# pocokhc/simple_distributed_rl

Measured on AMD Instinct MI355X. Metric: env-steps/sec + learner updates/sec, Rainbow 84x84x4, higher is better.
Workload: dtype f32

## Files before the change

### simple_distributed_rl_amd/csrc/srlx_qnet_bwd.hip

```cpp
#include <new>

#include "srlx_adam_math.h"
#include "srlx_qnet_int.h"
#include "srlx_td_math.h"

namespace {

using i64 = int64_t;
using u8 = unsigned char;
using f32x16 = __attribute__((ext_vector_type(16))) float;

constexpr int kFcSplits = 16;
constexpr int kWgSplits = 64;
constexpr int kC1Pad = 88, kC1Frame = kC1Pad * kC1Pad, kC1Chunks = 4;

__device__ __forceinline__ int clampi(int v, int lo, int hi) { return v < lo ? lo : (v > hi ? hi : v); }
__device__ __forceinline__ float byte_to_unit(unsigned b) {
    const float x = (float)b, rcp = 1.0f / 255.0f;
    const float q = x * rcp;
    return fmaf(fmaf(-q, 255.0f, x), rcp, q);
}

template <int AMAX>
__global__ void __launch_bounds__(256) k_head_bwd(int B, i64 sstride, int hidden, int A, int dueling, const float *dq,
                                                   const float *__restrict__ h1, const float *__restrict__ v2w, const float *__restrict__ a2w,
                                                   float *__restrict__ dh1, float *__restrict__ dh1t , float *__restrict__ g_bf,
                                                   float *__restrict__ g_v2w, float *__restrict__ g_v2b, float *__restrict__ g_a2w, float *__restrict__ g_a2b,
                                                   srlx::TdArgs td, int with_td) {
    extern __shared__ __attribute__((aligned(16))) float sm[];
    float *dv = sm, *da = sm + B, *part = sm + B + B * A;
    if (with_td) {
        float *sdq = part + (3 + AMAX) * 256;
        int off = B + 2 * B * A + (3 + AMAX) * 256;
        off += off & 1;
        double *red = reinterpret_cast<double *>(sm + off);
        const int t = threadIdx.x;
        const double la = srlx::td_rows(td, t, 256, sdq, blockIdx.x == 0);
        if (blockIdx.x == 0) {
            red[t] = la;
            __syncthreads();
            for (int s = 128; s > 0; s >>= 1) {
                if (t < s) red[t] += red[t + s];
                __syncthreads();
            }
            if (t == 0) td.loss[0] = (float)(red[0] / (double)td.B);
        }
        __syncthreads();
        dq = sdq;
    }
    for (int b = threadIdx.x; b < B; b += blockDim.x) {
        float s = 0.f;
        for (int j = 0; j < A; j++) s += dq[b * A + j];
        dv[b] = s;
        for (int j = 0; j < A; j++) da[b * A + j] = dueling == 0 ? dq[b * A + j] - s / (float)A : dq[b * A + j];
    }
    __syncthreads();
    const int ul = threadIdx.x & 63, slice = threadIdx.x >> 6;
    const int u = blockIdx.x * 64 + ul;
    const int N1 = 2 * hidden;
    float gv = 0.f, gbv = 0.f, gba = 0.f, ga[AMAX];
#pragma unroll
    for (int j = 0; j < AMAX; j++) ga[j] = 0.f;
    if (u < hidden) {
        const float wv = v2w[u];
        float wa[AMAX];
#pragma unroll
        for (int j = 0; j < AMAX; j++) wa[j] = j < A ? a2w[j * hidden + u] : 0.f;
#pragma unroll 8
        for (int b = slice; b < B; b += 4) {
            const float hv = h1[(i64)b * sstride * N1 + u], ha = h1[(i64)b * sstride * N1 + hidden + u];
            gv += dv[b] * hv;
            float s = 0.f;
#pragma unroll
            for (int j = 0; j < AMAX; j++)
                if (j < A) {
                    ga[j] += da[b * A + j] * ha;
                    s += da[b * A + j] * wa[j];
                }
            const float dhv = hv > 0.f ? dv[b] * wv : 0.f, dha = ha > 0.f ? s : 0.f;
            dh1[(i64)b * N1 + u] = dhv;
            dh1[(i64)b * N1 + hidden + u] = dha;
            if (dh1t) dh1t[u * 32 + b] = dhv, dh1t[(hidden + u) * 32 + b] = dha;
            gbv += dhv;
            gba += dha;
        }
        if (dh1t)
            for (int b = slice; b < 32; b += 4)
                if (b >= B) dh1t[u * 32 + b] = 0.f, dh1t[(hidden + u) * 32 + b] = 0.f;
    }
    part[0 * 256 + threadIdx.x] = gv;
    part[1 * 256 + threadIdx.x] = gbv;
    part[2 * 256 + threadIdx.x] = gba;
#pragma unroll
    for (int j = 0; j < AMAX; j++)
        if (j < A) part[(3 + j) * 256 + threadIdx.x] = ga[j];
    __syncthreads();
    if (slice == 0 && u < hidden) {
        auto sum4 = [&](int row) { return ((part[row * 256 + ul] + part[row * 256 + 64 + ul]) + part[row * 256 + 128 + ul]) + part[row * 256 + 192 + ul]; };
        g_v2w[u] = sum4(0);
        g_bf[u] = sum4(1);
        g_bf[hidden + u] = sum4(2);
#pragma unroll
        for (int j = 0; j < AMAX; j++)
            if (j < A) g_a2w[j * hidden + u] = sum4(3 + j);
    }
    if (blockIdx.x == 0 && threadIdx.x <= A) {
        float s = 0.f;
        if (threadIdx.x == A) {
            for (int b = 0; b < B; b++) s += dv[b];
            g_v2b[0] = s;
        } else {
            for (int b = 0; b < B; b++) s += da[b * A + threadIdx.x];
            g_a2b[threadIdx.x] = s;
        }
    }
}

__global__ void __launch_bounds__(256) k_uvfa_wgrad(int B, i64 sstride, int N1, int X, srlx_uvfa_dev uv, const float *__restrict__ dh1, float *__restrict__ g_wx) {
    const int id = blockIdx.x * 256 + threadIdx.x;
    if (id >= X * N1) return;
    const int c = id / N1, u = id % N1;
    float s = 0.f;
    for (int b = 0; b < B; b++) {
        const i64 row = (i64)b * sstride;
        float x;
        if (c == uv.c_ext) x = uv.r_ext[row];
        else if (c == uv.c_int) x = uv.r_int[row];
        else if (uv.c_act >= 0 && c >= uv.c_act && c < uv.c_act + uv.n_act_in) x = uv.action[row] == c - uv.c_act ? 1.f : 0.f;
        else x = (uv.c_actor >= 0 && uv.actor[row] == c - uv.c_actor) ? 1.f : 0.f;
        s += dh1[(i64)b * N1 + u] * x;
    }
    g_wx[id] = s;
}

template <int AMAX>
__global__ void __launch_bounds__(256) k_head_plain_bwd(int B, i64 sstride, int N1, int A, const float *__restrict__ dq, const float *__restrict__ h1,
                                                         const float *__restrict__ w2, float *__restrict__ dh1, float *__restrict__ dh1t ,
                                                         float *__restrict__ g_bf, float *__restrict__ g_w2, float *__restrict__ g_b2, srlx::TdArgs td, int with_td) {
    extern __shared__ __attribute__((aligned(16))) float sm[];
    float *part = sm, *sdq = sm + (1 + AMAX) * 256;
    const int t = threadIdx.x;
    if (with_td) {
        int off = (1 + AMAX) * 256 + B * A;
        off += off & 1;
        double *red = reinterpret_cast<double *>(sm + off);
        const double la = srlx::td_rows(td, t, 256, sdq, blockIdx.x == 0);
        if (blockIdx.x == 0) {
            red[t] = la;
            __syncthreads();
            for (int s = 128; s > 0; s >>= 1) {
                if (t < s) red[t] += red[t + s];
                __syncthreads();
            }
            if (t == 0) td.loss[0] = (float)(red[0] / (double)td.B);
        }
// ... 9 lines not shown
    if (u < N1) {
        float wa[AMAX];
#pragma unroll
        for (int j = 0; j < AMAX; j++) wa[j] = j < A ? w2[(i64)j * N1 + u] : 0.f;
#pragma unroll 4
        for (int b = slice; b < B; b += 4) {
            const float hv = h1[(i64)b * sstride * N1 + u];
            float s = 0.f;
#pragma unroll
            for (int j = 0; j < AMAX; j++)
                if (j < A) {
                    const float d = sdq[b * A + j];
                    ga[j] += d * hv;
                    s += d * wa[j];
                }
            const float dh = hv > 0.f ? s : 0.f;
            dh1[(i64)b * N1 + u] = dh;
            if (dh1t) dh1t[u * 32 + b] = dh;
            gb += dh;
        }
        if (dh1t)
            for (int b = slice; b < 32; b += 4)
                if (b >= B) dh1t[u * 32 + b] = 0.f;
    }
    part[t] = gb;
#pragma unroll
    for (int j = 0; j < AMAX; j++)
        if (j < A) part[(1 + j) * 256 + t] = ga[j];
    __syncthreads();
    if (slice == 0 && u < N1) {
        auto sum4 = [&](int row) { return ((part[row * 256 + ul] + part[row * 256 + 64 + ul]) + part[row * 256 + 128 + ul]) + part[row * 256 + 192 + ul]; };
        g_bf[u] = sum4(0);
#pragma unroll
        for (int j = 0; j < AMAX; j++)
            if (j < A) g_w2[(i64)j * N1 + u] = sum4(1 + j);
    }
    if (blockIdx.x == 0 && t < A) {
        float s = 0.f;
        for (int b = 0; b < B; b++) s += sdq[b * A + t];
        g_b2[t] = s;
    }
}

__global__ void __launch_bounds__(256) k_hidden_bwd(int B, i64 sstride, int N1, int out_cols, const float *__restrict__ g, const float *__restrict__ h1,
                                                    float *__restrict__ dh1, float *__restrict__ dh1t, float *__restrict__ g_bf) {
    __shared__ float part[256];
    const int ul = threadIdx.x & 63, slice = threadIdx.x >> 6;
    const int u = blockIdx.x * 64 + ul;
    float gb = 0.f;
    if (u < N1) {
        for (int b = slice; b < B; b += 4) {
            const float hv = h1[(i64)b * sstride * N1 + u];
            const float d = (u < out_cols && hv > 0.f) ? g[(i64)b * out_cols + u] : 0.f;
            dh1[(i64)b * N1 + u] = d;
            if (dh1t) dh1t[u * 32 + b] = d;
            gb += d;
        }
        if (dh1t)
            for (int b = slice; b < 32; b += 4)
                if (b >= B) dh1t[u * 32 + b] = 0.f;
    }
    part[threadIdx.x] = gb;
    __syncthreads();
    if (slice == 0 && u < N1) g_bf[u] = ((part[ul] + part[64 + ul]) + part[128 + ul]) + part[192 + ul];
}

template <bool ADAM, bool PLANES = false>
__global__ void __launch_bounds__(256) k_fc1_wgrad(int B, i64 sstride, int N1, int K, const float *__restrict__ dh1, const float *__restrict__ act3,
                                                   float *__restrict__ g_wf, float *__restrict__ wf, float *__restrict__ m, float *__restrict__ v, double lr, double beta1,
                                                   double beta2, double eps, const i64 *__restrict__ d_step, _Float16 *__restrict__ planes = nullptr) {
    const int lane = threadIdx.x & 63, i = lane & 31, h = lane >> 5;
    const int k0 = (blockIdx.x * 4 + (threadIdx.x >> 6)) * 32, n0 = blockIdx.y * 32;
    if (k0 >= K) return;
    float pp[16], mm[16], vv[16];
    if (ADAM)
#pragma unroll
        for (int r = 0; r < 16; r++) {
            const i64 at = (i64)(n0 + (r & 3) + 8 * (r >> 2) + 4 * h) * K + k0 + i;
            pp[r] = wf[at], mm[r] = m[at], vv[r] = v[at];
        }
    f32x16 acc;
#pragma unroll
    for (int r = 0; r < 16; r++) acc[r] = 0.f;
    const float *pa = dh1 + (i64)h * N1 + n0 + i, *pb = act3 + (i64)h * sstride * K + k0 + i;
    const int steps = (B + 1) / 2;
    for (int s0 = 0; s0 < steps; s0 += 8) {
        float av[8], bv[8];
#pragma unroll
        for (int q = 0; q < 8; q++) {
            const bool live = 2 * (s0 + q) + h < B;
            av[q] = live ? pa[(i64)(s0 + q) * 2 * N1] : 0.f;
            bv[q] = live ? pb[(i64)(s0 + q) * 2 * sstride * K] : 0.f;
        }
#pragma unroll
        for (int q = 0; q < 8; q++) acc = __builtin_amdgcn_mfma_f32_32x32x2f32(av[q], bv[q], acc, 0, 0, 0);
    }
    if (ADAM) {
        const srlx::AdamCoef c = srlx::adam_coef(lr, beta1, beta2, eps, *d_step);
#pragma unroll
        for (int r = 0; r < 16; r++) {
            const i64 at = (i64)(n0 + (r & 3) + 8 * (r >> 2) + 4 * h) * K + k0 + i;
            srlx::adam_one(pp[r], acc[r], mm[r], vv[r], c);
            wf[at] = pp[r], m[at] = mm[r], v[at] = vv[r];
            if (PLANES) {
                _Float16 *row = planes + (((i64)(k0 >> 5) * N1 + n0 + (r & 3) + 8 * (r >> 2) + 4 * h) * 64) + i;
                const _Float16 hi = (_Float16)pp[r];
                row[0] = hi;
                row[32] = (_Float16)((pp[r] - (float)hi) * 2048.0f);
            }
        }
    } else {
#pragma unroll
        for (int r = 0; r < 16; r++) g_wf[(i64)(n0 + (r & 3) + 8 * (r >> 2) + 4 * h) * K + k0 + i] = acc[r];
    }
}

template <int BT>
__global__ void __launch_bounds__(256) k_fc1_dgrad(int B, int N1, int K, const float *__restrict__ dh1, const float *__restrict__ wf, float *__restrict__ part) {
    __shared__ float sd[BT * 64];
    const int per = N1 / kFcSplits;
    const int n0 = blockIdx.y * per;
    const int k = blockIdx.x * 256 + threadIdx.x;
    for (int idx = threadIdx.x; idx < BT * per; idx += 256) {
        const int b = idx / per, nn = idx % per;
        sd[b * 64 + nn] = b < B ? dh1[(i64)b * N1 + n0 + nn] : 0.f;
    }
    __syncthreads();
    if (k >= K) return;
    float acc[BT];
#pragma unroll
    for (int b = 0; b < BT; b++) acc[b] = 0.f;
#pragma unroll 8
    for (int nn = 0; nn < per; nn++) {
        const float w = wf[(i64)(n0 + nn) * K + k];
#pragma unroll
        for (int b = 0; b < BT; b++) acc[b] += sd[b * 64 + nn] * w;
    }
#pragma unroll
    for (int b = 0; b < BT; b++)
        if (b < B) part[((i64)blockIdx.y * B + b) * K + k] = acc[b];
}

__global__ void __launch_bounds__(256) k_fc1_dgrad_reduce(int B, i64 sstride, int K, const float *__restrict__ part, const float *__restrict__ act3,
                                                          float *__restrict__ dact3) {
    const unsigned i = blockIdx.x * 256u + threadIdx.x;
    if (i >= (unsigned)(B * K)) return;
    const int b = (int)(i / (unsigned)K), k = (int)(i % (unsigned)K);
    float s = 0.f;
#pragma unroll
    for (int sp = 0; sp < kFcSplits; sp++) s += part[((i64)sp * B + b) * K + k];
    dact3[i] = act3[(i64)b * sstride * K + k] > 0.f ? s : 0.f;
}

__global__ void __launch_bounds__(256) k_fc1_dgrad_mfma(int B, i64 sstride, int N1, int K, const float *__restrict__ dh1t, const float *__restrict__ wf,
                                                        const float *__restrict__ act3, float *__restrict__ dact3) {
    __shared__ float red[3][16][64];
    const int t = threadIdx.x, wave = t >> 6, lane = t & 63, i = lane & 31, h = lane >> 5;
    const int k0 = blockIdx.x * 32;
    const int per = N1 / 4;
    const float *pa = dh1t + ((i64)wave * per + h) * 32 + i;
    const float *pb = wf + ((i64)wave * per + h) * K + k0 + i;
    f32x16 acc;
#pragma unroll
    for (int r = 0; r < 16; r++) acc[r] = 0.f;
    float a0[8], b0[8], a1[8], b1[8];
    auto fetch = [&](float *a, float *b, int s0) {
#pragma unroll
        for (int q = 0; q < 8; q++) {
            a[q] = pa[(i64)(s0 + q) * 64];
            b[q] = pb[(i64)(s0 + q) * 2 * K];
        }
    };
    const int steps = per / 2;
    fetch(a0, b0, 0);
    for (int s0 = 0; s0 < steps; s0 += 16) {
        if (s0 + 8 < steps) fetch(a1, b1, s0 + 8);
        __builtin_amdgcn_sched_barrier(0);
#pragma unroll
        for (int q = 0; q < 8; q++) acc = __builtin_amdgcn_mfma_f32_32x32x2f32(a0[q], b0[q], acc, 0, 0, 0);
        __builtin_amdgcn_sched_barrier(0);
        if (s0 + 8 >= steps) break;
        if (s0 + 16 < steps) fetch(a0, b0, s0 + 16);
        __builtin_amdgcn_sched_barrier(0);
#pragma unroll
        for (int q = 0; q < 8; q++) acc = __builtin_amdgcn_mfma_f32_32x32x2f32(a1[q], b1[q], acc, 0, 0, 0);
        __builtin_amdgcn_sched_barrier(0);
    }
    if (wave > 0)
#pragma unroll
        for (int r = 0; r < 16; r++) red[wave - 1][r][lane] = acc[r];
    __syncthreads();
    if (wave == 0)
#pragma unroll
        for (int r = 0; r < 16; r++) {
            const int b = (r & 3) + 8 * (r >> 2) + 4 * h;
            if (b < B) {
                const float sum = ((acc[r] + red[0][r][lane]) + red[1][r][lane]) + red[2][r][lane];
                dact3[(i64)b * K + k0 + i] = act3[(i64)b * sstride * K + k0 + i] > 0.f ? sum : 0.f;
            }
        }
}

struct ConvGeo {
    int H, W, CI, OH, OW, CO, KH, KW, S, P;
};
template <int CI>
__global__ void __launch_bounds__(256) k_conv_wgrad_mfma(ConvGeo g, i64 sstride, const float *__restrict__ X, const float *__restrict__ dY, float *__restrict__ part,
                                                         float *__restrict__ bias_part ) {
    constexpr int NCI = CI / 32, CO = 64;
    const int lane = threadIdx.x & 63, i = lane & 31, h = lane >> 5;
    const int combo = blockIdx.x * 4 + (threadIdx.x >> 6), taps = g.KH * g.KW;
    if (combo >= taps * 2 * NCI) return;
    const int cit = combo % NCI, cot = (combo / NCI) & 1, tap = combo / (2 * NCI);
    const int ky = tap / g.KW, kx = tap % g.KW;
    const i64 b = blockIdx.y;
    const int per_img = g.OH * g.OW, steps = (per_img + 1) / 2;
    const float *pa = dY + b * per_img * CO + cot * 32 + i;
    const float *px = X + b * sstride * g.H * g.W * CI + cit * 32 + i;
    int m = h, oy = 0, ox = h;
    f32x16 acc;
#pragma unroll
    for (int r = 0; r < 16; r++) acc[r] = 0.f;
    float bsum = 0.f;
    float a0[8], x0[8], a1[8], x1[8];
    auto fetch = [&](float *a, float *x) __attribute__((always_inline)) {
#pragma unroll
        for (int q = 0; q < 8; q++) {
            const bool live = m < per_img;
            const int iy = clampi(oy * g.S + ky - g.P, 0, g.H - 1), ix = clampi(ox * g.S + kx - g.P, 0, g.W - 1);
            a[q] = live ? pa[(i64)m * CO] : 0.f;
            x[q] = live ? px[((i64)iy * g.W + ix) * CI] : 0.f;
            m += 2, ox += 2;
            if (ox >= g.OW) ox -= g.OW, oy++;
        }
    };
    auto mfma8 = [&](const float *a, const float *x) __attribute__((always_inline)) {
#pragma unroll
        for (int q = 0; q < 8; q++) {
            bsum += a[q];
            acc = __builtin_amdgcn_mfma_f32_32x32x2f32(a[q], x[q], acc, 0, 0, 0);
        }
    };
    fetch(a0, x0);
    for (int s0 = 0; s0 < steps; s0 += 16) {
        if (s0 + 8 < steps) fetch(a1, x1);
        __builtin_amdgcn_sched_barrier(0);
        mfma8(a0, x0);
        __builtin_amdgcn_sched_barrier(0);
        if (s0 + 8 >= steps) break;
        if (s0 + 16 < steps) fetch(a0, x0);
        __builtin_amdgcn_sched_barrier(0);
        mfma8(a1, x1);
        __builtin_amdgcn_sched_barrier(0);
    }
#pragma unroll
    for (int r = 0; r < 16; r++) {
        const int co = cot * 32 + (r & 3) + 8 * (r >> 2) + 4 * h;
        part[((b * CO + co) * taps + tap) * CI + cit * 32 + i] = acc[r];
    }
    if (tap == 0 && cit == 0) {
        const float tot = bsum + __shfl_xor(bsum, 32);
        if (h == 0) bias_part[b * CO + cot * 32 + i] = tot;
    }
}

struct AdamArgs {
    double lr, beta1, beta2, eps;
    const i64 *d_step;
};
template <bool ADAM>
__global__ void __launch_bounds__(256) k_reduce_parts(const float *__restrict__ part, int P, i64 n, float *__restrict__ out, const float *__restrict__ bpart, int nb,
                                                      float *__restrict__ bout, float *__restrict__ pw = nullptr, float *__restrict__ mw = nullptr,
                                                      float *__restrict__ vw = nullptr, float *__restrict__ pb = nullptr, float *__restrict__ mb = nullptr,
                                                      float *__restrict__ vb = nullptr, AdamArgs ad = AdamArgs{}, i64 *__restrict__ snap = nullptr) {
    __shared__ float4 sm[4][64];
    const int lane = threadIdx.x & 63, sl = threadIdx.x >> 6;
    i64 i = ((i64)blockIdx.x * 64 + lane) * 4;
    const bool live = i < n + nb;
    if (ADAM && snap && blockIdx.x == 0 && threadIdx.x == 0) *snap = *ad.d_step;
    if (i >= n) {
        i -= n;
        part = bpart;
        n = nb;
        out = bout;
        pw = pb, mw = mb, vw = vb;
    }
    float4 pp, mm, vv;
    i64 step = 0;
    if (ADAM && sl == 0 && live) {
        pp = *reinterpret_cast<const float4 *>(pw + i), mm = *reinterpret_cast<const float4 *>(mw + i), vv = *reinterpret_cast<const float4 *>(vw + i);
        step = *ad.d_step;
    }
    const int per = (P + 3) / 4, p_lo = sl * per, p_hi = p_lo + per < P ? p_lo + per : P;
    float4 s = make_float4(0.f, 0.f, 0.f, 0.f);
    if (live)
#pragma unroll 8
        for (int p = p_lo; p < p_hi; p++) {
            const float4 v = *reinterpret_cast<const float4 *>(part + (i64)p * n + i);
            s.x += v.x, s.y += v.y, s.z += v.z, s.w += v.w;
        }
    sm[sl][lane] = s;
    __syncthreads();
    if (sl == 0 && live) {
        const float4 a = sm[1][lane], b = sm[2][lane], c = sm[3][lane];
        const float4 g = make_float4(((s.x + a.x) + b.x) + c.x, ((s.y + a.y) + b.y) + c.y, ((s.z + a.z) + b.z) + c.z, ((s.w + a.w) + b.w) + c.w);
        *reinterpret_cast<float4 *>(out + i) = g;
        if (ADAM) {
            const srlx::AdamCoef cf = srlx::adam_coef(ad.lr, ad.beta1, ad.beta2, ad.eps, step);
            srlx::adam_one(pp.x, g.x, mm.x, vv.x, cf);
            srlx::adam_one(pp.y, g.y, mm.y, vv.y, cf);
            srlx::adam_one(pp.z, g.z, mm.z, vv.z, cf);
            srlx::adam_one(pp.w, g.w, mm.w, vv.w, cf);
            *reinterpret_cast<float4 *>(pw + i) = pp;
            *reinterpret_cast<float4 *>(mw + i) = mm;
            *reinterpret_cast<float4 *>(vw + i) = vv;
        }
    }
}

__global__ void __launch_bounds__(256) k_transpose_filter(const float *__restrict__ W, int CO, int KH, int KW, int S, int CI, float *__restrict__ wT) {
    const int i = blockIdx.x * 256 + threadIdx.x;
    const int taps = KH * KW;
    if (i >= CO * taps * CI) return;
    const int ci = i % CI, tap = (i / CI) % taps, co = i / (CI * taps);
    const int ky = tap / KW, kx = tap % KW, KWS = KW / S, Kc = (KH / S) * KWS * CO;
    const int cls = (ky % S) * S + (kx % S);
    wT[((i64)cls * CI + ci) * Kc + ((ky / S) * KWS + kx / S) * CO + co] = W[i];
}

__global__ void __launch_bounds__(256) k_fold_pad(int B, i64 sstride, int H, int W, int CI, int P, int HP, int WP, int S, int QH, int QW,
                                                  const float *__restrict__ dxq, const float *__restrict__ X, float *__restrict__ dX, int nsplit = 1, i64 split_stride = 0) {
    const unsigned i4 = blockIdx.x * 256u + threadIdx.x;
    const unsigned c4n = (unsigned)CI / 4u;
    if (i4 >= (unsigned)(B * H * W) * c4n) return;
    const unsigned uw = (unsigned)W, uh = (unsigned)H;
    const int ci = 4 * (int)(i4 % c4n), ix = (int)((i4 / c4n) % uw), iy = (int)((i4 / (c4n * uw)) % uh), b = (int)(i4 / (c4n * uw * uh));
    const int y0 = iy == 0 ? 0 : iy + P, y1 = iy == H - 1 ? HP - 1 : iy + P;
    const int x0 = ix == 0 ? 0 : ix + P, x1 = ix == W - 1 ? WP - 1 : ix + P;
    const i64 cls_stride = (i64)B * QH * QW * CI;
    float4 s = make_float4(0.f, 0.f, 0.f, 0.f);
    for (int py = y0; py <= y1; py++)
        for (int px = x0; px <= x1; px++) {
            const float *src = dxq + ((py % S) * S + px % S) * cls_stride + (((i64)b * QH + py / S) * QW + px / S) * CI + ci;
            float4 v = *reinterpret_cast<const float4 *>(src);
            for (int sp = 1; sp < nsplit; sp++) {
                const float4 w = *reinterpret_cast<const float4 *>(src + sp * split_stride);
                v.x += w.x, v.y += w.y, v.z += w.z, v.w += w.w;
            }
            s.x += v.x, s.y += v.y, s.z += v.z, s.w += v.w;
        }
    const float4 x = *reinterpret_cast<const float4 *>(X + (((i64)b * sstride * H + iy) * W + ix) * CI + ci);
    *reinterpret_cast<float4 *>(dX + (i64)i4 * 4) = make_float4(x.x > 0.f ? s.x : 0.f, x.y > 0.f ? s.y : 0.f, x.z > 0.f ? s.z : 0.f, x.w > 0.f ? s.w : 0.f);
}

// ... 253 lines not shown
}

static int conv_chain(srlx_qnet_t *h, int B, i64 ss, const uint8_t *d_frame_base, const int64_t *d_frame_off, float *const *g, hipStream_t st, bool with_fc1) {
    const int N1 = 2 * h->hidden, K = h->flat, C2 = 2 * h->F1;
    float *g_w1 = g[0], *g_b1 = g[1], *g_w2 = g[2], *g_b2 = g[3], *g_w3 = g[4], *g_b3 = g[5], *g_wf = with_fc1 ? g[6] : nullptr;
    float *bias_part = h->w_part + h->w_part_floats;
    const size_t c3 = (size_t)2 * h->F1 * 9 * 2 * h->F1, c2 = (size_t)2 * h->F1 * 16 * h->F1;
    hipStream_t sd = h->side;
    SRLX_HIP(hipEventRecord(h->ev_d3, st));
    {
        const int HP = h->OH2 + 2, WP = h->OW2 + 2;
        const int nsplit = (C2 == 64 && h->dgrad_split == 2) ? 2 : 1;
        SRLX_TRY(srlx_qnet_dgrad_gemm(h->dact3, B, HP, WP, h->OH3, h->OW3, C2, 3, 3, 1, h->w_t, C2, h->dxpad, st, nsplit));
        const i64 tot = (i64)B * h->OH2 * h->OW2 * C2;
        hipLaunchKernelGGL(k_fold_pad, dim3((unsigned)((tot / 4 + 255) / 256)), dim3(256), 0, st, B, ss, h->OH2, h->OW2, C2, 1, HP, WP, 1, HP, WP, h->dxpad, h->act2, h->dact2, nsplit,
                           (i64)B * HP * WP * C2);
    }
    SRLX_STAMP(18, st);
    SRLX_HIP(hipEventRecord(h->ev_d2, st));
    {
        const int HP = h->OH1 + 4, WP = h->OW1 + 4, QH = (HP + 1) / 2, QW = (WP + 1) / 2;
        SRLX_TRY(srlx_qnet_dgrad_gemm(h->dact2, B, QH, QW, h->OH2, h->OW2, C2, 4, 4, 2, h->w_t2, h->F1, h->dxpad, st));
        const i64 tot = (i64)B * h->OH1 * h->OW1 * h->F1;
        hipLaunchKernelGGL(k_fold_pad, dim3((unsigned)((tot / 4 + 255) / 256)), dim3(256), 0, st, B, ss, h->OH1, h->OW1, h->F1, 2, HP, WP, 2, QH, QW, h->dxpad, h->act1, h->dact1);
    }
    SRLX_STAMP(19, st);
    SRLX_HIP(hipEventRecord(h->ev_d1, st));
    const dim3 fg((unsigned)((K / 32 + 3) / 4), (unsigned)(N1 / 32));
    if (with_fc1 && !h->adam_m)
        hipLaunchKernelGGL(k_fc1_wgrad<false>, fg, dim3(256), 0, sd, B, ss, N1, K, h->dh1, h->act3, g_wf, nullptr, nullptr, nullptr, 0.0, 0.0, 0.0, 0.0, nullptr);
    SRLX_HIP(hipStreamWaitEvent(sd, h->ev_d3, 0));
    const int fc1_order = h->fc1_order;
    auto launch_fc1_adam = [&](hipStream_t s2) {
        if (h->adam_planes_out)
            hipLaunchKernelGGL((k_fc1_wgrad<true, true>), fg, dim3(256), 0, s2, B, ss, N1, K, h->dh1, h->act3, nullptr, const_cast<float *>(h->wf), h->adam_m, h->adam_v,
                               h->adam_lr, h->adam_b1, h->adam_b2, h->adam_eps, h->adam_step, (_Float16 *)h->adam_planes_out);
        else
            hipLaunchKernelGGL(k_fc1_wgrad<true>, fg, dim3(256), 0, s2, B, ss, N1, K, h->dh1, h->act3, nullptr, const_cast<float *>(h->wf), h->adam_m, h->adam_v, h->adam_lr,
                               h->adam_b1, h->adam_b2, h->adam_eps, h->adam_step);
    };
    const bool fc1_adam = with_fc1 && h->adam_m;
    if (fc1_adam && fc1_order == 1) launch_fc1_adam(sd);
    if (fc1_adam && fc1_order == 2) {
        if (!h->side2) SRLX_HIP(hipStreamCreateWithFlags(&h->side2, hipStreamNonBlocking));
        SRLX_HIP(hipStreamWaitEvent(h->side2, h->ev_d3, 0));
        launch_fc1_adam(h->side2);
        SRLX_HIP(hipEventRecord(h->ev_join2, h->side2));
    }
    ConvGeo g3{h->OH2, h->OW2, C2, h->OH3, h->OW3, C2, 3, 3, 1, 1};
    hipLaunchKernelGGL(k_conv_wgrad_mfma<64>, dim3((9 * 2 * 2 + 3) / 4, (unsigned)B), dim3(256), 0, sd, g3, ss, h->act2, h->dact3, h->w_part, bias_part);
    const bool rest = h->rest_on && with_fc1;
    const AdamArgs ad{h->adam_lr, h->adam_b1, h->adam_b2, h->adam_eps, h->adam_step};
    auto reduce = [&](hipStream_t s_, const float *part_, int P_, i64 n_, float *gw_, const float *bp_, int nb_, float *gb_, int wi, i64 *snap_) {
        const dim3 grid((unsigned)((n_ + nb_ + 255) / 256));
        if (rest)
            hipLaunchKernelGGL(k_reduce_parts<true>, grid, dim3(256), 0, s_, part_, P_, n_, gw_, bp_, nb_, gb_, const_cast<float *>(h->bound[wi]), h->rest_m[wi], h->rest_v[wi],
                               const_cast<float *>(h->bound[wi + 1]), h->rest_m[wi + 1], h->rest_v[wi + 1], ad, snap_);
        else
            hipLaunchKernelGGL(k_reduce_parts<false>, grid, dim3(256), 0, s_, part_, P_, n_, gw_, bp_, nb_, gb_);
    };
    reduce(sd, h->w_part, B, (i64)C2 * 9 * C2, g_w3, bias_part, C2, g_b3, 4, nullptr);
    SRLX_STAMP(22, sd);
    SRLX_HIP(hipStreamWaitEvent(sd, h->ev_d2, 0));
    ConvGeo g2{h->OH1, h->OW1, h->F1, h->OH2, h->OW2, C2, 4, 4, 2, 2};
    hipLaunchKernelGGL(k_conv_wgrad_mfma<32>, dim3((16 * 2 * 1 + 3) / 4, (unsigned)B), dim3(256), 0, sd, g2, ss, h->act1, h->dact2, h->w_part, bias_part);
    reduce(sd, h->w_part, B, (i64)C2 * 16 * h->F1, g_w2, bias_part, C2, g_b2, 2, nullptr);
    SRLX_STAMP(23, sd);
    if (fc1_adam && fc1_order != 1 && fc1_order != 2) launch_fc1_adam(sd);
    SRLX_STAMP(24, sd);
    SRLX_HIP(hipEventRecord(h->ev_join, sd));
    constexpr int c1_chunks = 2;
    constexpr bool c1_in_launch = false;
    const int per = ((h->OH1 * h->OW1 + c1_chunks - 1) / c1_chunks + 1) & ~1;
    const size_t lds = (size_t)kC1Frame + (size_t)per * 4 + (size_t)per * 32 * sizeof(float) + 2 * 16 * 64 * sizeof(float);
    SRLX_REQUIRE(lds <= 64 * 1024, "qnet_backward_u8: conv1 staging needs %zu bytes of LDS", lds);
    float *c1_part = h->w_part + kWgSplits * (c3 > c2 ? c3 : c2), *c1_bias = bias_part + 2 * kWgSplits * 64;
    hipLaunchKernelGGL(k_conv1_wgrad_mfma, dim3((unsigned)B, (unsigned)(c1_chunks * h->Wn)), dim3(256), lds, st, d_frame_base, d_frame_off, ss, h->Wn, h->H, h->W, h->OH1, h->OW1, per,
                       h->dact1, c1_part, c1_bias, h->c1_gpart, h->c1_cnt, g_w1, g_b1, c1_chunks, c1_in_launch ? 1 : 0);
    if (!c1_in_launch)
        reduce(st, c1_part, B * c1_chunks, (i64)32 * h->Wn * 64, g_w1, c1_bias, 32, g_b1, 0, h->step_snap);
    SRLX_STAMP(20, st);
    SRLX_HIP(hipStreamWaitEvent(st, h->ev_join, 0));
    if (fc1_adam && fc1_order == 2) SRLX_HIP(hipStreamWaitEvent(st, h->ev_join2, 0));
    return SRLX_OK;
}

__global__ void __launch_bounds__(256) k_relu_mask_rows(const float *__restrict__ gy, const float *__restrict__ act, i64 ss, i64 row, i64 total, float *__restrict__ out) {
    const i64 q = (i64)blockIdx.x * blockDim.x + threadIdx.x;
    if (q * 4 >= total) return;
    const i64 b = (q * 4) / row, k = (q * 4) % row;
    const float4 gv = *reinterpret_cast<const float4 *>(gy + q * 4), a = *reinterpret_cast<const float4 *>(act + b * ss * row + k);
    *reinterpret_cast<float4 *>(out + q * 4) = make_float4(a.x > 0.f ? gv.x : 0.f, a.y > 0.f ? gv.y : 0.f, a.z > 0.f ? gv.z : 0.f, a.w > 0.f ? gv.w : 0.f);
}

static int backward_impl(srlx_qnet_t *h, int64_t batch, int64_t sample_stride, const uint8_t *d_frame_base, const int64_t *d_frame_off, const float *d_grad_q,
                         const srlx::TdArgs *td, float *const *g, void *stream) {
    SRLX_REQUIRE(h && d_frame_base && d_frame_off && (d_grad_q || td) && g, "qnet_backward_u8: NULL argument");
    SRLX_REQUIRE(h->max_train > 0, "qnet_backward_u8: call srlx_qnet_enable_training first");
    SRLX_REQUIRE(batch > 0 && batch <= h->max_train && sample_stride >= 1 && batch * sample_stride <= h->max_batch, "qnet_backward_u8: batch %lld x stride %lld out of range",
                 (long long)batch, (long long)sample_stride);
    for (int i = 0; i < 12; i++) SRLX_REQUIRE(g[i], "qnet_backward_u8: gradient buffer %d is NULL", i);
    SRLX_REQUIRE(!h->sig[0] || h->g_sig[0], "qnet_backward_u8: the network is noisy but no sigma gradient tensors are bound (srlx_qnet_bind_noisy_grads)");
    if (h->rest_on) {
        SRLX_REQUIRE(!h->rest_armed, "qnet_backward_u8: the previous pass's optimiser step was never completed (srlx_qnet_publish must follow every backward pass "
                                     "of a handle with srlx_qnet_fuse_adam_rest)");
        for (int i = 7; i < 12; i++) SRLX_REQUIRE(g[i] == h->rest_g[i], "qnet_backward_u8: gradient buffer %d is not the one srlx_qnet_fuse_adam_rest was given", i);
    }
    srlx::DeviceGuard guard(h->device);
    hipStream_t st = (hipStream_t)stream;
    const int B = (int)batch, N1 = 2 * h->hidden, K = h->flat, A = h->A;
    const i64 ss = sample_stride;
    float *g_bf = g[7], *g_v2w = g[8], *g_v2b = g[9], *g_a2w = g[10], *g_a2b = g[11];

    const bool mfma_dgrad = B <= 32;
    if (h->head_mode == 1) {
        SRLX_REQUIRE(!td && !h->ln_w, "qnet_backward_u8: a hidden-layer handle takes the gradient of its output (no TD prologue, no LayerNorm inside)");
        hipLaunchKernelGGL(k_hidden_bwd, dim3((unsigned)((N1 + 63) / 64)), dim3(256), 0, st, B, ss, N1, h->out_cols, d_grad_q, h->h1, h->dh1, mfma_dgrad ? h->dh1t : nullptr, g_bf);
    } else if (h->dueling == kHeadPlain) {
        const int amax = A <= 8 ? 8 : (A <= 16 ? 16 : 32);
        const size_t hl = (size_t)((1 + amax) * 256 + B * A + 2 + (td ? 512 : 0)) * sizeof(float);
        float *dh1t = mfma_dgrad ? h->dh1t : nullptr;
        const srlx::TdArgs tda = td ? *td : srlx::TdArgs{};
        const int with_td = td ? 1 : 0;
        const dim3 hg((unsigned)((N1 + 63) / 64));
        if (A <= 8)
            hipLaunchKernelGGL(k_head_plain_bwd<8>, hg, dim3(256), hl, st, B, ss, N1, A, d_grad_q, h->h1, h->a2w, h->dh1, dh1t, g_bf, g_a2w, g_a2b, tda, with_td);
        else if (A <= 16)
            hipLaunchKernelGGL(k_head_plain_bwd<16>, hg, dim3(256), hl, st, B, ss, N1, A, d_grad_q, h->h1, h->a2w, h->dh1, dh1t, g_bf, g_a2w, g_a2b, tda, with_td);
        else
            hipLaunchKernelGGL(k_head_plain_bwd<32>, hg, dim3(256), hl, st, B, ss, N1, A, d_grad_q, h->h1, h->a2w, h->dh1, dh1t, g_bf, g_a2w, g_a2b, tda, with_td);
    } else {
        const dim3 hg((unsigned)((h->hidden + 63) / 64));
        const size_t hl = (size_t)(B + B * A + (3 + (A <= 8 ? 8 : (A <= 16 ? 16 : 32))) * 256 + (td ? B * A + 2 + 512 : 0)) * sizeof(float);
        float *dh1t = mfma_dgrad ? h->dh1t : nullptr;
        const srlx::TdArgs tda = td ? *td : srlx::TdArgs{};
        const int with_td = td ? 1 : 0;
        if (A <= 8)
            hipLaunchKernelGGL(k_head_bwd<8>, hg, dim3(256), hl, st, B, ss, h->hidden, A, h->dueling, d_grad_q, h->h1, h->v2w, h->a2w, h->dh1, dh1t, g_bf, g_v2w, g_v2b, g_a2w,
                               g_a2b, tda, with_td);
        else if (A <= 16)
            hipLaunchKernelGGL(k_head_bwd<16>, hg, dim3(256), hl, st, B, ss, h->hidden, A, h->dueling, d_grad_q, h->h1, h->v2w, h->a2w, h->dh1, dh1t, g_bf, g_v2w, g_v2b, g_a2w,
                               g_a2b, tda, with_td);
        else
            hipLaunchKernelGGL(k_head_bwd<32>, hg, dim3(256), hl, st, B, ss, h->hidden, A, h->dueling, d_grad_q, h->h1, h->v2w, h->a2w, h->dh1, dh1t, g_bf, g_v2w, g_v2b, g_a2w,
                               g_a2b, tda, with_td);
    }
    SRLX_STAMP(16, st);
    if (h->ev_td) SRLX_HIP(hipEventRecord(h->ev_td, st));
    const bool main_first = h->main_first;
    const bool uvfa = h->uvfa.X > 0;
    SRLX_REQUIRE(!uvfa || h->uvfa.g_wx, "qnet_backward_u8: a UVFA network needs a gradient buffer for its columns (srlx_qnet_fuse_adam_uvfa)");
    SRLX_TRY(chain_prologue(h, st, main_first && mfma_dgrad ? 1 : 3, uvfa, B, ss));
    if (mfma_dgrad) {
        hipLaunchKernelGGL(k_fc1_dgrad_mfma, dim3((unsigned)(K / 32)), dim3(256), 0, st, B, ss, N1, K, h->dh1t, h->wf, h->act3, h->dact3);
        if (main_first) SRLX_TRY(chain_prologue(h, st, 2, uvfa, B, ss));
    } else {
        hipLaunchKernelGGL(k_fc1_dgrad<64>, dim3((unsigned)((K + 255) / 256), kFcSplits), dim3(256), 0, st, B, N1, K, h->dh1, h->wf, h->fc_part);
        hipLaunchKernelGGL(k_fc1_dgrad_reduce, dim3((unsigned)(((i64)B * K + 255) / 256)), dim3(256), 0, st, B, ss, K, h->fc_part, h->act3, h->dact3);
    }
    SRLX_STAMP(17, st);
    SRLX_TRY(conv_chain(h, B, ss, d_frame_base, d_frame_off, g, st, true));
    SRLX_TRY(srlx_qnet_noisy_sigma_grads(h, g, st));
    SRLX_HIP(hipGetLastError());
    h->rest_armed = h->rest_on;
    return SRLX_OK;
}

int srlx_qnet_backward_u8(srlx_qnet_t *h, int64_t batch, int64_t sample_stride, const uint8_t *d_frame_base, const int64_t *d_frame_off,
                          const float *d_grad_q, float *const *g, void *stream) {
    SRLX_REQUIRE(d_grad_q, "qnet_backward_u8: NULL argument");
    return backward_impl(h, batch, sample_stride, d_frame_base, d_frame_off, d_grad_q, nullptr, g, stream);
}

int srlx_qnet_backward_convs_u8(srlx_qnet_t *h, int64_t batch, int64_t sample_stride, const uint8_t *d_frame_base, const int64_t *d_frame_off, const float *d_grad_features,
                                float *const *g, void *stream) {
    SRLX_REQUIRE(h && d_frame_base && d_frame_off && d_grad_features && g, "qnet_backward_convs_u8: NULL argument");
    SRLX_REQUIRE(h->max_train > 0, "qnet_backward_convs_u8: call srlx_qnet_enable_training first");
    SRLX_REQUIRE(batch > 0 && batch <= h->max_train && sample_stride >= 1 && batch * sample_stride <= h->max_batch, "qnet_backward_convs_u8: batch %lld x stride %lld out of range",
                 (long long)batch, (long long)sample_stride);
    for (int i = 0; i < 6; i++) SRLX_REQUIRE(g[i], "qnet_backward_convs_u8: gradient buffer %d is NULL", i);
    srlx::DeviceGuard guard(h->device);
    hipStream_t st = (hipStream_t)stream;
    SRLX_TRY(chain_prologue(h, st));
    const i64 total = (i64)batch * h->flat;
    hipLaunchKernelGGL(k_relu_mask_rows, dim3((unsigned)((total / 4 + 255) / 256)), dim3(256), 0, st, d_grad_features, h->act3, (i64)sample_stride, (i64)h->flat, total, h->dact3);
    SRLX_TRY(conv_chain(h, (int)batch, (i64)sample_stride, d_frame_base, d_frame_off, g, st, false));
    SRLX_HIP(hipGetLastError());
    return SRLX_OK;
}

int srlx_qnet_backward_td_u8(srlx_qnet_t *h, int64_t batch, int n_step, const uint8_t *d_frame_base, const int64_t *d_frame_off, const float *d_q_on_all,
                             const float *d_q_tg_next, const int32_t *d_actions, const float *d_rewards, const float *d_terminated, const uint8_t *d_invalid_next,
                             const float *d_weights, double discount, double retrace_h, int enable_double_dqn, int enable_rescale, float *d_target, float *d_loss,
                             float *d_grad_q0, float *d_priorities, float *const *g, void *stream) {
    SRLX_REQUIRE(h, "qnet_backward_td_u8: NULL handle");
    SRLX_REQUIRE(batch > 0 && batch <= 256 && n_step >= 1 && n_step <= srlx::kTdMaxStep, "qnet_backward_td_u8: bad sizes (n_step <= %d)", srlx::kTdMaxStep);
    SRLX_REQUIRE(d_q_on_all && d_q_tg_next && d_actions && d_rewards && d_terminated && d_weights, "qnet_backward_td_u8: NULL input");
    SRLX_REQUIRE(d_target && d_loss && d_grad_q0 && d_priorities, "qnet_backward_td_u8: NULL output");
    const int A = h->A;
    const int64_t row = (int64_t)(n_step + 1) * A;
    srlx::TdArgs td{batch, n_step, A, d_q_on_all + A, d_q_tg_next, d_q_on_all, d_actions, d_rewards, d_terminated, d_invalid_next, d_weights, discount, retrace_h,
                          enable_double_dqn, enable_rescale, d_target, d_loss, d_grad_q0, d_priorities, row, row};
    srlx::td_fill_discounts(td);
    td.disc_ps = h->td_disc_ps, td.td_signed = h->td_signed;
    return backward_impl(h, batch, n_step + 1, d_frame_base, d_frame_off, nullptr, &td, g, stream);
}

}

namespace {

struct SeqGeo {
    int H, W, CI, OH, OW, KH, KW, S, P;
};
template <int NCI>
__global__ void __launch_bounds__(256) k_wgrad_seq(SeqGeo g, const float *__restrict__ X, const float *__restrict__ dY, float *__restrict__ part,
                                                   float *__restrict__ bias_part , i64 rows, int rpp) {
    constexpr bool kFrames = NCI == 0;
    constexpr int CO = kFrames ? 32 : 64;
    const int lane = threadIdx.x & 63, i = lane & 31, h = lane >> 5;
    const int combo = blockIdx.x * 4 + (threadIdx.x >> 6), taps = g.KH * g.KW;
    const int ncombo = kFrames ? 2 * g.CI : taps * 2 * NCI;
    if (combo >= ncombo) return;
    int ky, kx, cot = 0, xoff, tap = 0, cit = 0;
    if (kFrames) {
        const int k = combo * 32 + i;
        xoff = k >> 6, ky = (k & 63) >> 3, kx = k & 7;
    } else {
        cit = combo % (NCI ? NCI : 1), cot = (combo / (NCI ? NCI : 1)) & 1, tap = combo / (2 * (NCI ? NCI : 1));
        ky = tap / g.KW, kx = tap % g.KW, xoff = cit * 32 + i;
    }
    const i64 p = blockIdx.y, b_lo = p * rpp, b_hi = b_lo + rpp < rows ? b_lo + rpp : rows;
    const int per_img = g.OH * g.OW, steps = (per_img + 1) / 2;
    f32x16 acc;
#pragma unroll
    for (int r = 0; r < 16; r++) acc[r] = 0.f;
    float bsum = 0.f;
    for (i64 b = b_lo; b < b_hi; b++) {
        const float *pa = dY + b * per_img * CO + cot * 32 + i;
        const float *px = X + b * (i64)g.H * g.W * g.CI + xoff;
        int m = h, oy = 0, ox = h;
        float a0[8], x0[8], a1[8], x1[8];
        auto fetch = [&](float *a, float *x) __attribute__((always_inline)) {
#pragma unroll
            for (int q = 0; q < 8; q++) {
                const bool live = m < per_img;
                const int iy = clampi(oy * g.S + ky - g.P, 0, g.H - 1), ix = clampi(ox * g.S + kx - g.P, 0, g.W - 1);
                a[q] = live ? pa[(i64)m * CO] : 0.f;
                x[q] = live ? px[((i64)iy * g.W + ix) * g.CI] : 0.f;
                m += 2, ox += 2;
                if (ox >= g.OW) ox -= g.OW, oy++;
            }
        };
        auto mfma8 = [&](const float *a, const float *x) __attribute__((always_inline)) {
#pragma unroll
            for (int q = 0; q < 8; q++) {
                bsum += a[q];
                acc = __builtin_amdgcn_mfma_f32_32x32x2f32(a[q], x[q], acc, 0, 0, 0);
            }
        };
        fetch(a0, x0);
        for (int s0 = 0; s0 < steps; s0 += 16) {
            if (s0 + 8 < steps) fetch(a1, x1);
            __builtin_amdgcn_sched_barrier(0);
            mfma8(a0, x0);
            __builtin_amdgcn_sched_barrier(0);
            if (s0 + 8 >= steps) break;
            if (s0 + 16 < steps) fetch(a0, x0);
            __builtin_amdgcn_sched_barrier(0);
            mfma8(a1, x1);
            __builtin_amdgcn_sched_barrier(0);
        }
    }
#pragma unroll
    for (int r = 0; r < 16; r++) {
        const int co = cot * 32 + (r & 3) + 8 * (r >> 2) + 4 * h;
        if (kFrames)
            part[(p * CO + co) * ((i64)g.CI * 64) + combo * 32 + i] = acc[r];
        else
            part[((p * CO + co) * taps + tap) * g.CI + cit * 32 + i] = acc[r];
    }
    if (kFrames ? combo == 0 : (tap == 0 && cit == 0)) {
        const float tot = bsum + __shfl_xor(bsum, 32);
        if (h == 0) bias_part[p * CO + cot * 32 + i] = tot;
    }
}

__global__ void __launch_bounds__(256) k_seq_grad_in(const float *__restrict__ gy, i64 ld, const float *__restrict__ act3, int P, int CH, float *__restrict__ dact3) {
    extern __shared__ float tr[];
    const i64 r = blockIdx.x;
    const int flat = P * CH;
    const float *src = gy + r * ld;
    for (int idx = threadIdx.x; idx < flat; idx += 256) tr[(idx % P) * (CH + 1) + idx / P] = src[idx];
    __syncthreads();
    for (int idx = threadIdx.x; idx < flat; idx += 256) dact3[r * flat + idx] = act3[r * flat + idx] > 0.f ? tr[(idx / CH) * (CH + 1) + idx % CH] : 0.f;
}

struct SeqSizes {
    size_t dact3, dact2, dact1, dxpad, w_t, w_t2, w_part, part_stride;
    size_t bytes() const { return (dact3 + dact2 + dact1 + dxpad + w_t + w_t2 + w_part) * sizeof(float); }
};
bool seq_sizes(int H, int W, int C, int F1, i64 rows, SeqSizes *z) {
    if (F1 != 32 || H != W || H % 4 != 0 || H < 8 || H > 84 || C < 1 || C > 4 || rows < 1 || rows > kSeqMaxRows) return false;
    const size_t OH1 = (size_t)(H + 6 - 8) / 4 + 1, OH2 = (OH1 + 4 - 4) / 2 + 1, OH3 = OH2, R = (size_t)rows;
    z->dact3 = R * OH3 * OH3 * 64, z->dact2 = R * OH2 * OH2 * 64, z->dact1 = R * OH1 * OH1 * 32;
    const size_t q = (OH1 + 5) / 2, pad2 = 4 * q * q * 32, pad3 = (OH2 + 2) * (OH2 + 2) * 64;
    z->dxpad = R * (pad2 > pad3 ? pad2 : pad3) + 128 * 64;
// ... 93 lines not shown
```

Before: 2.156 million.

## Pipeline fc1 dgrad MFMA loads through a register ring with LDS-staged A operand

Rewrites the fc1 data-gradient MFMA kernel so global loads run through a compile-time ring of NB chunks (depth 4) instead of a two-buffer ping-pong. The A operand (dh1t) is fetched as 16-byte vector loads and redistributed through per-wave LDS double buffers. The ReLU mask from act3 is prefetched into registers before the main loop. The aim is to hide global-load latency behind the MFMAs and cut load instruction count. In exchange it uses more registers and adds LDS traffic and wave barriers.

Result: slower. 2.130 million (-1.2%).

```diff
diff --git a/simple_distributed_rl_amd/csrc/srlx_fc1_dgrad_mfma.h b/simple_distributed_rl_amd/csrc/srlx_fc1_dgrad_mfma.h
--- /dev/null
+++ b/simple_distributed_rl_amd/csrc/srlx_fc1_dgrad_mfma.h
@@ -0,0 +1,119 @@
+#pragma once
+#include <stdint.h>
+
+#include <type_traits>
+#include <utility>
+
+#include <hip/hip_runtime.h>
+
+namespace srlx {
+
+template <int I0, int... I, class F>
+__device__ __forceinline__ void static_for_seq(std::integer_sequence<int, I...>, F &&f) {
+    (f(std::integral_constant<int, I0 + I>{}), ...);
+}
+template <int I0, int I1, class F>
+__device__ __forceinline__ void static_for(F &&f) {
+    static_for_seq<I0>(std::make_integer_sequence<int, I1 - I0>{}, f);
+}
+
+template <int NB>
+__global__ void __launch_bounds__(256) k_fc1_dgrad_mfma(int B, int64_t sstride, int N1, int K, const float *__restrict__ dh1t, const float *__restrict__ wf,
+                                                        const float *__restrict__ act3, float *__restrict__ dact3) {
+    static_assert(NB >= 2 && 10 * NB <= 63, "ring depth: ten loads per chunk, the vmcnt counter holds 63");
+    using f32x16 = __attribute__((ext_vector_type(16))) float;
+    using f32x4 = __attribute__((ext_vector_type(4))) float;
+    using i64 = int64_t;
+    __shared__ __attribute__((aligned(16))) float sm[4][2 * 512];
+    const int t = threadIdx.x, wave = t >> 6, lane = t & 63, i = lane & 31, h = lane >> 5;
+    const int k0 = blockIdx.x * 32;
+    const int per = N1 / 4;
+    const int nch = per / 16;
+    const f32x4 *pa = reinterpret_cast<const f32x4 *>(dh1t + (i64)wave * per * 32) + lane;
+    const float *pb = wf + ((i64)wave * per + h) * K + k0 + i;
+    float *sw = sm[wave];
+    f32x16 acc;
+#pragma unroll
+    for (int r = 0; r < 16; r++) acc[r] = 0.f;
+    f32x4 a[NB][2];
+    float b[NB][8];
+    float relu[16];
+    if (wave == 0)
+#pragma unroll
+        for (int r = 0; r < 16; r++) {
+            const int bb = (r & 3) + 8 * (r >> 2) + 4 * h;
+            relu[r] = act3[(i64)(bb < B ? bb : B - 1) * sstride * K + k0 + i];
+        }
+    auto fetch = [&](f32x4 *as, float *bs, int c) __attribute__((always_inline)) {
+#pragma unroll
+        for (int q = 0; q < 8; q++) bs[q] = pb[(i64)(c * 8 + q) * 2 * K];
+        const int ca = c + 1 < nch ? c + 1 : nch - 1;
+        as[0] = pa[ca * 128];
+        as[1] = pa[ca * 128 + 64];
+    };
+    auto mul = [&](const f32x4 *as, const float *bs, int c) __attribute__((always_inline)) {
+        f32x4 *wr = reinterpret_cast<f32x4 *>(sw + ((c + 1) & 1) * 512) + lane;
+        __builtin_amdgcn_wave_barrier();
+        wr[0] = as[0];
+        wr[64] = as[1];
+        __builtin_amdgcn_wave_barrier();
+        const float *rd = sw + (c & 1) * 512 + lane;
+        float av[8];
+#pragma unroll
+        for (int q = 0; q < 8; q++) av[q] = rd[q * 64];
+#pragma unroll
+        for (int q = 0; q < 8; q++) acc = __builtin_amdgcn_mfma_f32_32x32x2f32(av[q], bs[q], acc, 0, 0, 0);
+    };
+    {
+        const f32x4 a00 = pa[0], a01 = pa[64];
+#pragma unroll
+        for (int j = 0; j < NB - 1; j++) fetch(a[j], b[j], j < nch ? j : nch - 1);
+        f32x4 *wr = reinterpret_cast<f32x4 *>(sw) + lane;
+        wr[0] = a00;
+        wr[64] = a01;
+    }
+    __builtin_amdgcn_sched_barrier(0);
+    int c = 0;
+    auto step = [&](auto J) __attribute__((always_inline)) {
+        constexpr int j = decltype(J)::value % NB, jn = (j + NB - 1) % NB;
+        fetch(a[jn], b[jn], c + NB - 1);
+        __builtin_amdgcn_sched_barrier(0);
+        mul(a[j], b[j], c);
+        __builtin_amdgcn_sched_barrier(0);
+        c++;
+    };
+    auto drain = [&](auto J) __attribute__((always_inline)) {
+        constexpr int j = decltype(J)::value % NB;
+        if (c < nch) {
+            mul(a[j], b[j], c);
+            __builtin_amdgcn_sched_barrier(0);
+            c++;
+        }
+    };
+    const int steady = nch > NB - 1 ? nch - (NB - 1) : 0;
+    for (int turns = steady / NB; turns > 0; turns--) static_for<0, NB>(step);
+    const int rem = steady % NB;
+    static_for<0, NB>([&](auto R) __attribute__((always_inline)) {
+        constexpr int r = decltype(R)::value;
+        if (rem == r) {
+            static_for<0, r>(step);
+            static_for<r, r + NB - 1>(drain);
+        }
+    });
+    __builtin_amdgcn_wave_barrier();
+    if (wave > 0)
+#pragma unroll
+        for (int r = 0; r < 16; r++) sw[r * 64 + lane] = acc[r];
+    __syncthreads();
+    if (wave == 0)
+#pragma unroll
+        for (int r = 0; r < 16; r++) {
+            const int bb = (r & 3) + 8 * (r >> 2) + 4 * h;
+            if (bb < B) {
+                const float sum = ((acc[r] + sm[1][r * 64 + lane]) + sm[2][r * 64 + lane]) + sm[3][r * 64 + lane];
+                dact3[(i64)bb * K + k0 + i] = relu[r] > 0.f ? sum : 0.f;
+            }
+        }
+}
+
+}
diff --git a/simple_distributed_rl_amd/csrc/srlx_qnet_bwd.hip b/simple_distributed_rl_amd/csrc/srlx_qnet_bwd.hip
--- a/simple_distributed_rl_amd/csrc/srlx_qnet_bwd.hip
+++ b/simple_distributed_rl_amd/csrc/srlx_qnet_bwd.hip
@@ -1,6 +1,7 @@
 #include <new>
 
 #include "srlx_adam_math.h"
+#include "srlx_fc1_dgrad_mfma.h"
 #include "srlx_qnet_int.h"
 #include "srlx_td_math.h"
 
@@ -316,54 +317,7 @@
     dact3[i] = act3[(i64)b * sstride * K + k] > 0.f ? s : 0.f;
 }
 
-__global__ void __launch_bounds__(256) k_fc1_dgrad_mfma(int B, i64 sstride, int N1, int K, const float *__restrict__ dh1t, const float *__restrict__ wf,
-                                                        const float *__restrict__ act3, float *__restrict__ dact3) {
-    __shared__ float red[3][16][64];
-    const int t = threadIdx.x, wave = t >> 6, lane = t & 63, i = lane & 31, h = lane >> 5;
-    const int k0 = blockIdx.x * 32;
-    const int per = N1 / 4;
-    const float *pa = dh1t + ((i64)wave * per + h) * 32 + i;
-    const float *pb = wf + ((i64)wave * per + h) * K + k0 + i;
-    f32x16 acc;
-#pragma unroll
-    for (int r = 0; r < 16; r++) acc[r] = 0.f;
-    float a0[8], b0[8], a1[8], b1[8];
-    auto fetch = [&](float *a, float *b, int s0) {
-#pragma unroll
-        for (int q = 0; q < 8; q++) {
-            a[q] = pa[(i64)(s0 + q) * 64];
-            b[q] = pb[(i64)(s0 + q) * 2 * K];
-        }
-    };
-    const int steps = per / 2;
-    fetch(a0, b0, 0);
-    for (int s0 = 0; s0 < steps; s0 += 16) {
-        if (s0 + 8 < steps) fetch(a1, b1, s0 + 8);
-        __builtin_amdgcn_sched_barrier(0);
-#pragma unroll
-        for (int q = 0; q < 8; q++) acc = __builtin_amdgcn_mfma_f32_32x32x2f32(a0[q], b0[q], acc, 0, 0, 0);
-        __builtin_amdgcn_sched_barrier(0);
-        if (s0 + 8 >= steps) break;
-        if (s0 + 16 < steps) fetch(a0, b0, s0 + 16);
-        __builtin_amdgcn_sched_barrier(0);
-#pragma unroll
-        for (int q = 0; q < 8; q++) acc = __builtin_amdgcn_mfma_f32_32x32x2f32(a1[q], b1[q], acc, 0, 0, 0);
-        __builtin_amdgcn_sched_barrier(0);
-    }
-    if (wave > 0)
-#pragma unroll
-        for (int r = 0; r < 16; r++) red[wave - 1][r][lane] = acc[r];
-    __syncthreads();
-    if (wave == 0)
-#pragma unroll
-        for (int r = 0; r < 16; r++) {
-            const int b = (r & 3) + 8 * (r >> 2) + 4 * h;
-            if (b < B) {
-                const float sum = ((acc[r] + red[0][r][lane]) + red[1][r][lane]) + red[2][r][lane];
-                dact3[(i64)b * K + k0 + i] = act3[(i64)b * sstride * K + k0 + i] > 0.f ? sum : 0.f;
-            }
-        }
-}
+constexpr int kFc1DgradRing = 4;
 
 struct ConvGeo {
     int H, W, CI, OH, OW, CO, KH, KW, S, P;
@@ -923,7 +877,7 @@
     SRLX_REQUIRE(!uvfa || h->uvfa.g_wx, "qnet_backward_u8: a UVFA network needs a gradient buffer for its columns (srlx_qnet_fuse_adam_uvfa)");
     SRLX_TRY(chain_prologue(h, st, main_first && mfma_dgrad ? 1 : 3, uvfa, B, ss));
     if (mfma_dgrad) {
-        hipLaunchKernelGGL(k_fc1_dgrad_mfma, dim3((unsigned)(K / 32)), dim3(256), 0, st, B, ss, N1, K, h->dh1t, h->wf, h->act3, h->dact3);
+        hipLaunchKernelGGL(srlx::k_fc1_dgrad_mfma<kFc1DgradRing>, dim3((unsigned)(K / 32)), dim3(256), 0, st, B, ss, N1, K, h->dh1t, h->wf, h->act3, h->dact3);
         if (main_first) SRLX_TRY(chain_prologue(h, st, 2, uvfa, B, ss));
     } else {
         hipLaunchKernelGGL(k_fc1_dgrad<64>, dim3((unsigned)((K + 255) / 256), kFcSplits), dim3(256), 0, st, B, N1, K, h->dh1, h->wf, h->fc_part);
```
